# lesliegaga/GPT-SoVITS

Hardware: AMD Instinct MI355X
Metric: synthesised audio sec/sec (1/RTF), v2 pipeline (higher is better)
Workload: dtype f16

## Files before the change

gpt-sovits_amd/csrc/attn.hip:

```cpp
#include <stdlib.h>

#include "common.h"

#define GSV_PIN() do { asm volatile("" ::: "memory"); __builtin_amdgcn_sched_barrier(0); } while (0)

namespace gsv {

__device__ __forceinline__ f4 mma16(h8 a, h8 b, f4 c) { return __builtin_amdgcn_mfma_f32_16x16x32_f16(a, b, c, 0, 0, 0); }

__global__ __launch_bounds__(256) void vt_kernel(const _Float16* __restrict__ v, int ld, int T, int ldv, _Float16* __restrict__ vt,
                                                 int heads, _Float16* __restrict__ q, int ldq, _Float16* __restrict__ k, int ldk,
                                                 const float* __restrict__ rope_cs, int rope_half, int planes, long long xz,
                                                 long long vtz) {
  const int row = blockIdx.z / planes, plane = blockIdx.z - row * planes;
  v += row * xz; q += row * xz; k += row * xz; vt += row * vtz;
  if (plane == heads) {
    const int n = T * rope_half * 2;
    const int stride = gridDim.x * gridDim.y * 256;
    for (int i = (blockIdx.y * gridDim.x + blockIdx.x) * 256 + threadIdx.x; i < n; i += stride) {
      const int which = i / (T * rope_half);
      const int rr = i - which * T * rope_half;
      const int t = rr / rope_half, p = rr - t * rope_half;
      _Float16* x = (which ? k + (long long)t * ldk : q + (long long)t * ldq) + 2 * p;
      const float c = rope_cs[((long long)t * rope_half + p) * 2], sn = rope_cs[((long long)t * rope_half + p) * 2 + 1];
// ... 315 lines not shown
      den += e * Ls[w * BQ + qq];
      acc += *(const f4*)&Os[((size_t)w * BQ + qq) * LDO + d4] * e;
    }
#pragma unroll
    for (int rr = 0; rr < NB; ++rr) {
      const float pw = __expf(Sb[qq * NB + rr] - mt);
      const f4 rv = *(const f4*)(rel_v + rr * D + d4);
      acc += rv * pw;
    }
    const float inv = 1.f / den;
    *(h4*)(out + (long long)(q0 + qq) * ldo + head * D + d4) =
        (h4){(_Float16)(acc[0] * inv), (_Float16)(acc[1] * inv), (_Float16)(acc[2] * inv), (_Float16)(acc[3] * inv)};
  }
}

int launch_flash_rel96_f16(const void* q, int ldq, const void* k, int ldk, const void* v, int ldvv, void* vt_buf, int T, int heads,
                           float scale, const float* rel_k, const float* rel_v, void* out, int ldo, hipStream_t s, const int* kr) {
  GSV_REQUIRE(T >= 1 && heads >= 1 && rel_k && rel_v, "flash_rel96: bad argument");
  GSV_REQUIRE(ldq % 8 == 0 && ldk % 8 == 0 && ldo % 4 == 0 && ((uintptr_t)q % 16) == 0 && ((uintptr_t)k % 16) == 0 && ((uintptr_t)out % 8) == 0 &&
              ((uintptr_t)rel_v % 16) == 0, "flash_rel96: operands must be 16-byte aligned with leading dims multiple of 8");
  const int ldv = (T + 31) / 32 * 32;
  hipLaunchKernelGGL(vt96_kernel, dim3(ldv / 32, 3, heads), dim3(256), 0, s, (const _Float16*)v, ldvv, T, ldv, (_Float16*)vt_buf);
  constexpr int QT = 2;
  const size_t lds = ((size_t)4 * 16 * QT * 100 + 8 * 16 * QT + 2 * 16 * QT * 9) * 4;
  static bool attr = false;
  if (!attr) {
    GSV_HIP(hipFuncSetAttribute((const void*)flash_rel96_f16_kernel<QT>, hipFuncAttributeMaxDynamicSharedMemorySize, (int)lds));
    attr = true;
  }
  hipLaunchKernelGGL(flash_rel96_f16_kernel<QT>, dim3(cdiv(T, 16 * QT), heads), dim3(256), lds, s, (const _Float16*)q, ldq,
                     (const _Float16*)k, ldk, (const _Float16*)vt_buf, ldv, T, scale, rel_k, rel_v, (_Float16*)out, ldo, kr);
  GSV_HIP(hipGetLastError());
  return GSV_OK;
}

// ... 27 lines not shown
```

gpt-sovits_amd/csrc/engine.h:

```cpp
#pragma once
#include <math.h>
#include <map>
#include <string>
#include <vector>

#include "common.h"

struct Conv {
  void* w = nullptr;
  float* b = nullptr;
  int cin = 0, cout = 0, taps = 1;
  int ups_u = 0, ups_pad = 0, ups_cout = 0;
};

struct AttnLayerW { Conv qkv, o; float *rel_k = nullptr, *rel_v = nullptr; float *g1 = nullptr, *b1 = nullptr, *g2 = nullptr, *b2 = nullptr; Conv f1, f2; };
struct WNW { std::vector<Conv> in, res; std::vector<float*> in_bias_eff; Conv cond; };
struct FlowW { Conv pre, post; WNW wn; };

struct VocAct { float *alpha = nullptr, *beta = nullptr; };
struct GenW {
  int uic = 0, n_ups = 0, n_resblocks = 0;
  int up_rates[8], up_kernels[8], rb_kernels[4], rb_dilations[4][3];
  std::vector<Conv> ups, rb1, rb2;
  std::vector<VocAct> acts;
  int snake_logscale = 0;
  float *up12 = nullptr, *dn12 = nullptr;
};

struct Buf { void* p = nullptr; size_t cap = 0; };

struct gsv_vits {
  gsv_vits_config cfg;
// ... 91 lines not shown
```

gpt-sovits_amd/csrc/ops.hip:

```cpp
#include "common.h"

namespace gsv {

static thread_local char g_err[1024] = "";
void set_error(const char* fmt, ...) {
  va_list ap;
  va_start(ap, fmt);
  vsnprintf(g_err, sizeof(g_err), fmt, ap);
  va_end(ap);
}
const char* get_error() { return g_err; }

static thread_local unsigned long long g_conv_route = 0;
static thread_local unsigned long long g_pair_route = 0;
void set_conv_route(unsigned long long code) {
  g_conv_route = code;
  if ((code & 255) == ROUTE_CONV_PAIR) g_pair_route = code;
}

template <typename T> __global__ void convert_kernel(const float* __restrict__ s, T* __restrict__ d, long long n) {
  long long i = (long long)blockIdx.x * blockDim.x + threadIdx.x;
  long long stride = (long long)gridDim.x * blockDim.x;
  for (; i < n; i += stride) d[i] = (T)s[i];
}
// ... 219 lines not shown
                     float eps, int dtype, gsv_stream_t stream) {
  return gsv::launch_layernorm(dtype, x, 0, res, 0, gamma, beta, y, 0, rows, C, eps, (hipStream_t)stream);
}

int gsv_op_flash_attn64(const void* qkv, int T, int heads, float scale, void* vt_scratch, void* out, gsv_stream_t stream) {
  const int inner = heads * 64;
  return gsv::launch_flash_attn64_f16(qkv, 3 * inner, (const _Float16*)qkv + inner, 3 * inner, (const _Float16*)qkv + 2 * inner, 3 * inner,
                                      vt_scratch, T, heads, scale, out, inner, (hipStream_t)stream);
}

int gsv_op_flash_rel96(const void* qkv, int T, int heads, float scale, const float* rel_k, const float* rel_v, void* vt_scratch,
                       void* out, gsv_stream_t stream) {
  const int H = heads * 96;
  return gsv::launch_flash_rel96_f16(qkv, 3 * H, (const _Float16*)qkv + H, 3 * H, (const _Float16*)qkv + 2 * H, 3 * H, vt_scratch, T, heads,
                                     scale, rel_k, rel_v, out, H, (hipStream_t)stream);
}

int gsv_op_conv1d(const gsv_conv_desc* d, int dtype, gsv_stream_t stream) {
  gsv::ConvArgs a;
  a.x = d->x; a.w = d->w; a.bias = d->bias; a.y = d->y; a.res = d->res; a.gate = d->gate;
  a.T_in = d->T_in; a.T_out = d->T_out; a.Cin = d->Cin; a.Cout = d->Cout; a.taps = d->taps;
  a.stride = d->stride; a.dil = d->dil; a.pad = d->pad;
  a.ldx = d->Cin; a.ldw = d->taps * d->Cin;
  a.pre_act = d->pre_act; a.pre_slope = d->pre_slope; a.post_act = d->post_act; a.scale = d->scale;
  a.accumulate = d->accumulate; a.out_f32 = d->out_f32;
  a.res_f32 = d->res_dtype == 0 ? d->out_f32 : d->res_dtype == 1;
  a.y_col0 = d->y_col0; a.w_nt = d->w_nt; a.z_res = d->z_res;
  if (d->ups_u > 0) {
    a.ups_u = d->ups_u; a.ups_pad = d->ups_pad; a.ups_cout = d->Cout / d->ups_u;
    a.ldy = a.ups_cout; a.ldr = a.ups_cout;
// ... 88 lines not shown
```

gpt-sovits_amd/csrc/vits.hip:

```cpp
#include "engine.h"

namespace gsv {

template <typename T>
__global__ void gather_rows_kernel(const int* __restrict__ idx, const float* __restrict__ table, int C, int rep, int n,
                                   T* __restrict__ out) {
  const int row = blockIdx.x;
  if (row >= n * rep) return;
  const float* src = table + (long long)idx[row / rep] * C;
  T* dst = out + (long long)row * C;
  for (int c = threadIdx.x; c < C; c += blockDim.x) dst[c] = (T)src[c];
}

template <typename T>
__global__ void gather_seg_kernel(const int* __restrict__ ids, const int* __restrict__ src, const float* __restrict__ table, int C,
                                  int rows, T* __restrict__ out) {
  const int row = blockIdx.x;
  if (row >= rows) return;
  const int i = src[row];
  T* dst = out + (long long)row * C;
  if (i < 0) { for (int c = threadIdx.x; c < C; c += blockDim.x) dst[c] = (T)0.f; return; }
  const float* sp = table + (long long)ids[i] * C;
  for (int c = threadIdx.x; c < C; c += blockDim.x) dst[c] = (T)sp[c];
}
// ... 170 lines not shown
__global__ void gate_kernel(const T* __restrict__ a, long long n, int H, T* __restrict__ out) {
  long long i = (long long)blockIdx.x * blockDim.x + threadIdx.x;
  if (i >= n) return;
  long long t = i / H; int c = (int)(i - t * H);
  float x = to_f(a[t * 2 * H + c]), y = to_f(a[t * 2 * H + H + c]);
  out[i] = (T)(tanhf(x) * (1.f / (1.f + expf(-y))));
}

template <typename T>
__global__ void glu_res_kernel(const T* __restrict__ y, long long n, int H, T* __restrict__ x) {
  long long i = (long long)blockIdx.x * blockDim.x + threadIdx.x;
  if (i >= n) return;
  long long t = i / H; int c = (int)(i - t * H);
  float a = to_f(y[t * 2 * H + c]), b = to_f(y[t * 2 * H + H + c]);
  x[i] = (T)(to_f(x[i]) + a * (1.f / (1.f + expf(-b))));
}

template <typename T>
__global__ void flip_channels_kernel(const T* __restrict__ src, long long n, int C, T* __restrict__ dst) {
  long long i = (long long)blockIdx.x * blockDim.x + threadIdx.x;
  if (i >= n) return;
  long long t = i / C; int c = (int)(i - t * C);
  dst[i] = src[t * C + (C - 1 - c)];
}

__device__ __forceinline__ unsigned long long mix64(unsigned long long x) {
  x += 0x9E3779B97F4A7C15ull;
  x = (x ^ (x >> 30)) * 0xBF58476D1CE4E5B9ull;
  x = (x ^ (x >> 27)) * 0x94D049BB133111EBull;
  return x ^ (x >> 31);
}

template <typename T>
__global__ void zp_kernel(const float* __restrict__ stats, int F, int C, const float* __restrict__ noise, float scale,
                          unsigned long long seed, T* __restrict__ z, const int* __restrict__ seg, const int* __restrict__ start,
                          const int* __restrict__ noff, const unsigned long long* __restrict__ seeds, int Fn) {
  long long i = (long long)blockIdx.x * blockDim.x + threadIdx.x;
  if (i >= (long long)F * C) return;
// ... 646 lines not shown
  {
    std::vector<float> e;
    if (!fetch(h, "quantizer.vq.layers.0._codebook.embed", (size_t)c.n_bins * SSL, c.n_bins, e)) return GSV_ERR_ARG;
    GSV_RC(up_f32(h, e.data(), e.size(), &h->codebook));
    GSV_RC(up_t(h, e, &h->codebook_t));
    std::vector<float> ee(c.n_bins);
    for (int j = 0; j < c.n_bins; ++j) {
      float s = 0.f;
      for (int k = 0; k < SSL; ++k) s += e[(size_t)j * SSL + k] * e[(size_t)j * SSL + k];
      ee[j] = s;
    }
    GSV_RC(up_f32(h, ee.data(), ee.size(), &h->code_ee));
    GSV_RC(make_conv(h, "ssl_proj", SSL, SSL, 2, true, &h->top_ssl_proj));
  }
  if (c.flavor == 0) {
    for (int fi = 0; fi < 4; ++fi) {
      FlowW& f = h->flows[fi];
      const std::string p = "flow.flows." + std::to_string(2 * fi);
      GSV_RC(make_conv(h, p + ".pre", H, IC / 2, 1, true, &f.pre));
      GSV_RC(make_conv(h, p + ".post", IC / 2, H, 1, true, &f.post));
      GSV_RC(make_wn(h, p + ".enc", 4, H, GIN, &f.wn));
    }
    const int UIC = c.upsample_initial_channel;
    GSV_RC(make_conv(h, "dec.conv_pre", UIC, IC, 7, true, &h->conv_pre));
    GSV_RC(make_conv(h, "dec.cond", UIC, GIN, 1, true, &h->cond));
    GSV_RC(dalloc(h, (void**)&h->conv_pre_bias_eff, (size_t)UIC * 4));
    gen_shape(c, &h->gen);
    GSV_RC(load_generator(h, "dec.", false, &h->gen));
    GSV_RC(make_conv(h, "dec.conv_post", 1, UIC >> c.n_ups, 7, false, &h->conv_post));
  } else {
    const int W = 512, NL = 8;
    GSV_REQUIRE(IC == H, "vits: v3/v4 need inter_channels == hidden_channels (bridge = Conv1d(inter, 512) on the hidden sequence)");
    GSV_RC(make_conv(h, "bridge.0", W, IC, 1, true, &h->bridge));
    GSV_RC(make_conv(h, "wns1.pre", W, W, 1, true, &h->w1_pre));
    GSV_RC(make_conv(h, "wns1.proj", W, W, 1, true, &h->w1_proj));
// ... 65 lines not shown
}

template <typename T>
static int decode_wav(gsv_vits* h, hipStream_t s, const int32_t* codes, int Tc, const int32_t* phones, int L, double speed,
                      const float* noise, float noise_scale, uint64_t seed, float* wav, const SegRun* sr) {
  const auto& c = h->cfg;
  void* y = nullptr;
  int F = 0;
  GSV_RC(run_enc_p<T>(h, s, codes, Tc, phones, L, speed, &y, &F, sr));
  const size_t es = sizeof(T);
  const int H = c.hidden_channels, IC = c.inter_channels;
  const int* seg_f = sr ? sr->seg_p : nullptr;
  float* stats;
  GSV_RC(need(h, "stats", (size_t)F * 2 * IC * 4, (void**)&stats));
  { ConvOpt of; of.out_f32 = 1; GSV_RC(conv(h, s, h->proj, y, H, F, stats, F, of)); }
  void *z, *zf, *hb, *xin, *acts, *wout;
  GSV_RC(need(h, "z", (size_t)F * IC * es, &z));
  GSV_RC(need(h, "zf", (size_t)F * IC * es, &zf));
  GSV_RC(need(h, "wn_h", (size_t)F * H * es, &hb));
  GSV_RC(need(h, "wn_xin", (size_t)F * 2 * H * es, &xin));
  GSV_RC(need(h, "wn_acts", (size_t)F * H * es, &acts));
  GSV_RC(need(h, "wn_out", (size_t)F * H * es, &wout));
  GSV_LAUNCH(zp_kernel<T>, dim3(nblk((long long)F * IC)), dim3(256), 0, s, stats, F, IC, noise, noise_scale, (unsigned long long)seed, (T*)z,
             seg_f, sr ? sr->start : nullptr, sr ? sr->noff : nullptr, sr ? sr->seeds : nullptr, sr ? sr->post->Fn : 0);
  const int half = IC / 2;
  for (int fi = 3; fi >= 0; --fi) {
    FlowW& f = h->flows[fi];
    GSV_LAUNCH(flip_channels_kernel<T>, dim3(nblk((long long)F * IC)), dim3(256), 0, s, (const T*)z, (long long)F * IC, IC, (T*)zf);
    std::swap(z, zf);
    ConvOpt om; om.row_seg = seg_f;
    GSV_RC(conv(h, s, f.pre, z, IC, F, hb, F, om));
    GSV_RC(run_wn<T>(h, s, f.wn, F, hb, xin, acts, wout, sr, h->voice_off_in + (size_t)fi * 4 * 2 * H, F));
    ConvOpt op; op.scale = -1.f; op.accumulate = 1; op.ldy = IC; op.y_col0 = half; op.row_seg = seg_f;
    GSV_RC(conv(h, s, f.post, wout, H, F, z, F, op));
  }
  h->lastF = F;
  {
    void* zkeep;
    GSV_RC(need(h, "z_keep", (size_t)F * IC * es, &zkeep));
    GSV_HIP(hipMemcpyAsync(zkeep, z, (size_t)F * IC * es, hipMemcpyDeviceToDevice, s));
  }
  GSV_HIP(hipEventRecord(h->ev[1], s));
  void* gb[5];
  GSV_RC(gen_buffers(h, h->gen, "g", F, gb));
  void* cur = gb[3];
  GSV_RC(conv_voice(h, s, h->conv_pre, z, F, cur, ConvOpt(), h->conv_pre_bias_eff, sr, h->voice_off_pre, seg_f));
  int Tn = F;
  GSV_RC(run_generator_stages(h, s, h->gen, gb, &cur, &Tn, seg_f ? sr->seg_up.data() : nullptr));
  float* wout_p = wav;
  if (seg_f) GSV_RC(need(h, "wav_pad", (size_t)Tn * 4, (void**)&wout_p));
  { ConvOpt op; op.pre_act = ACT_LRELU; op.pre_slope = 0.01f; op.post_act = ACT_TANH; op.out_f32 = 1;
    GSV_RC(conv(h, s, h->conv_post, cur, h->conv_post.cin, Tn, wout_p, Tn, op)); }
  if (seg_f) {
    const int up = Tn / F;
    GSV_RC(launch_compact_wav(s, wout_p, seg_f, up, (long long)sr->post->G * up, (long long)Tn, wav));
  }
// ... 75 lines not shown
  GSV_REQUIRE(h && h->finalized, "vits_decode: handle not finalized");
  GSV_REQUIRE(h->has_ref, "vits_decode: call gsv_vits_set_refer first");
  GSV_REQUIRE(codes && phones && wav && Tc >= 1 && L >= 1, "vits_decode: empty input (T=%d, L=%d)", Tc, L);
  hipStream_t s = (hipStream_t)stream;
  GSV_REQUIRE(speed > 0.0, "vits_decode: speed must be positive");
  GSV_REQUIRE(h->cfg.flavor == 0, "vits_decode: this handle is a v3/v4 model (use gsv_vits_decode_encp + gsv_cfm_inference + a vocoder)");
  GSV_HIP(hipEventRecord(h->ev[0], s));
  return GSV_WITH_T(h, decode_wav<T>(h, s, codes, Tc, phones, L, speed, noise, noise_scale, seed, wav, nullptr));
}

int gsv_vits_segment_gap(const gsv_vits_config* cfg) {
  if (!cfg || cfg->n_ups < 1 || cfg->n_ups > 8 || cfg->n_resblocks < 1 || cfg->n_resblocks > 4) return -1;
  return seg_gap(*cfg);
}

int gsv_vits_segment_map(const gsv_vits_config* cfg, int n, const int* code_lens, const int* phone_lens, int level, int32_t* seg,
                         int64_t cap, int64_t* rows) {
  return gsv_vits_segment_map_speed(cfg, n, code_lens, phone_lens, nullptr, level, seg, cap, rows);
}

int gsv_vits_segment_map_speed(const gsv_vits_config* cfg, int n, const int* code_lens, const int* phone_lens, const double* speeds,
                               int level, int32_t* seg, int64_t cap, int64_t* rows) {
  GSV_REQUIRE(cfg && rows && cfg->n_ups >= 1 && cfg->n_ups <= 8, "vits_segment_map: bad argument");
  GSV_REQUIRE(level >= -1 && level <= cfg->n_ups, "vits_segment_map: level %d outside [-1, %d]", level, cfg->n_ups);
  SegLayout lay;
  GSV_RC(seg_layout(*cfg, n, code_lens, phone_lens, speeds, &lay));
  long long up = 1;
  for (int i = 0; i < level; ++i) up *= cfg->up_rates[i];
  const long long nr = level < 0 ? lay.L : (long long)lay.F * up;
  *rows = nr;
// ... 169 lines not shown
  }
  GSV_REQUIRE(F > 0, "vits_debug_tensor: no decode yet");
  if (n == "gen_last_in") {
    const long long ne = (long long)h->dbg_last_T * h->dbg_last_C;
    GSV_REQUIRE(h->dbg_last_in && cap >= ne, "vits_debug_tensor: buffer too small");
    *numel = ne;
    return GSV_WITH_T(h, debug_cl_to_cf<T>(s, h->dbg_last_in, h->dbg_last_T, h->dbg_last_C, out));
  }
  GSV_REQUIRE(cap >= (int64_t)F * IC, "vits_debug_tensor: buffer too small");
  *numel = (int64_t)F * IC;
  if (n == "m_p" || n == "logs_p") {
    const float* st = (const float*)h->bufs["stats"].p;
    GSV_LAUNCH(cl_to_cf_kernel<float>, dim3(nblk((long long)F * IC)), dim3(256), 0, s, st, F, 2 * IC, n == "m_p" ? 0 : IC, IC, out);
    return GSV_OK;
  }
  if (n == "z") return GSV_WITH_T(h, debug_cl_to_cf<T>(s, h->bufs["z_keep"].p, F, IC, out));
  set_error("vits_debug_tensor: unknown tensor '%s' (ge, m_p, logs_p, z, gen_last_in)", name);
  return GSV_ERR_ARG;
}

}
```

gpt-sovits_amd/gsv/_lib.py:

```python
from __future__ import annotations

import ctypes as C
import os

HERE = os.path.dirname(os.path.abspath(__file__))
LIB_PATH = os.path.join(HERE, "libgsv_hip.so")

GSV_F32, GSV_F16 = 0, 1


class T2SConfig(C.Structure):
    _fields_ = [(n, C.c_int) for n in ("n_layer", "dim", "n_head", "ffn_dim", "vocab", "phoneme_vocab", "bert_dim")]


class SamplingParams(C.Structure):
    _fields_ = [("top_k", C.c_int), ("top_p", C.c_float), ("temperature", C.c_float),
                ("repetition_penalty", C.c_float), ("early_stop_num", C.c_int), ("eos_mask_steps", C.c_int),
                ("max_steps", C.c_int), ("seed", C.c_uint64)]


class RowSampling(C.Structure):
    _fields_ = [("top_k", C.c_int), ("top_p", C.c_float), ("temperature", C.c_float), ("repetition_penalty", C.c_float)]


# ... 74 lines not shown
    "gsv_vits_debug_tensor": (C.c_int, [C.c_void_p, C.c_char_p, C.c_void_p, C.c_int64, C.POINTER(C.c_int64),
                                        C.c_void_p]),
    "gsv_vits_last_timing": (C.c_int, [C.c_void_p, C.POINTER(C.c_float), C.POINTER(C.c_float)]),
    "gsv_vits_store_voice": (C.c_int, [C.c_void_p, C.c_int]),
    "gsv_vits_decode_segments": (C.c_int, [C.c_void_p, C.c_int, C.c_void_p, C.POINTER(C.c_int), C.c_void_p, C.POINTER(C.c_int),
                                           C.POINTER(C.c_int), C.POINTER(C.c_uint64), C.c_void_p, C.c_float, C.c_void_p,
                                           C.c_void_p]),
    "gsv_vits_decode_segments_speed": (C.c_int, [C.c_void_p, C.c_int, C.c_void_p, C.POINTER(C.c_int), C.c_void_p, C.POINTER(C.c_int),
                                                 C.POINTER(C.c_int), C.POINTER(C.c_uint64), C.POINTER(C.c_double), C.c_void_p,
                                                 C.c_float, C.c_void_p, C.c_void_p]),
    "gsv_vits_segment_gap": (C.c_int, [C.POINTER(VitsConfig)]),
    "gsv_vits_segment_map": (C.c_int, [C.POINTER(VitsConfig), C.c_int, C.POINTER(C.c_int), C.POINTER(C.c_int), C.c_int,
                                       C.POINTER(C.c_int32), C.c_int64, C.POINTER(C.c_int64)]),
    "gsv_vits_segment_map_speed": (C.c_int, [C.POINTER(VitsConfig), C.c_int, C.POINTER(C.c_int), C.POINTER(C.c_int),
                                             C.POINTER(C.c_double), C.c_int, C.POINTER(C.c_int32), C.c_int64, C.POINTER(C.c_int64)]),
    "gsv_vocoder_create": (C.c_int, [C.POINTER(VocoderConfig), C.c_int, C.POINTER(C.c_void_p)]),
    "gsv_vocoder_destroy": (None, [C.c_void_p]),
    "gsv_vocoder_load_tensor": (C.c_int, [C.c_void_p, C.c_char_p, C.c_void_p, C.c_int64]),
    "gsv_vocoder_finalize": (C.c_int, [C.c_void_p]),
    "gsv_vocoder_forward": (C.c_int, [C.c_void_p, C.c_void_p, C.c_int, C.c_void_p, C.c_void_p]),
    "gsv_vocoder_forward_segments": (C.c_int, [C.c_void_p, C.c_void_p, C.c_int, C.POINTER(C.c_int), C.c_void_p, C.c_void_p]),
    "gsv_vocoder_segment_gap": (C.c_int, [C.POINTER(VocoderConfig)]),
    "gsv_vocoder_segment_map": (C.c_int, [C.POINTER(VocoderConfig), C.c_int, C.POINTER(C.c_int), C.c_int, C.POINTER(C.c_int32),
                                          C.c_int64]),
    "gsv_cfm_create": (C.c_int, [C.POINTER(DitConfig), C.c_int, C.POINTER(C.c_void_p)]),
    "gsv_cfm_destroy": (None, [C.c_void_p]),
    "gsv_cfm_load_tensor": (C.c_int, [C.c_void_p, C.c_char_p, C.c_void_p, C.c_int64]),
    "gsv_cfm_finalize": (C.c_int, [C.c_void_p]),
    "gsv_cfm_inference": (C.c_int, [C.c_void_p, C.c_void_p, C.c_void_p, C.c_int, C.c_int, C.c_int, C.c_int, C.c_void_p,
                                    C.c_float, C.c_uint64, C.c_void_p, C.c_void_p]),
# ... 14 lines not shown
    "gsv_postprocess": (C.c_int, [C.POINTER(C.c_void_p), C.POINTER(C.c_int), C.c_int, C.c_int, C.c_int, C.c_void_p, C.c_void_p]),
    "gsv_postprocess_f32": (C.c_int, [C.POINTER(C.c_void_p), C.POINTER(C.c_int), C.c_int, C.c_int, C.c_int, C.c_void_p,
                                      C.c_void_p]),
    "gsv_bwe_create": (C.c_int, [C.POINTER(BweConfig), C.c_int, C.POINTER(C.c_void_p)]),
    "gsv_bwe_destroy": (None, [C.c_void_p]),
    "gsv_bwe_load_tensor": (C.c_int, [C.c_void_p, C.c_char_p, C.c_void_p, C.c_int64]),
    "gsv_bwe_finalize": (C.c_int, [C.c_void_p]),
    "gsv_bwe_out_len": (C.c_int, [C.c_void_p, C.c_int, C.c_int]),
    "gsv_bwe_forward": (C.c_int, [C.c_void_p, C.c_void_p, C.c_int, C.c_int, C.c_int, C.c_void_p, C.c_void_p]),
    "gsv_bwe_debug_tensor": (C.c_int, [C.c_void_p, C.c_char_p, C.c_void_p, C.c_int64, C.POINTER(C.c_int64), C.c_void_p]),
    "gsv_aa_act_forward": (C.c_int, [C.c_void_p, C.c_void_p, C.c_void_p, C.c_void_p, C.c_void_p, C.c_void_p,
                                     C.c_int, C.c_int, C.c_int, C.c_int, C.c_void_p]),
    "gsv_op_flash_attn64": (C.c_int, [C.c_void_p, C.c_int, C.c_int, C.c_float, C.c_void_p, C.c_void_p, C.c_void_p]),
    "gsv_op_flash_rel96": (C.c_int, [C.c_void_p, C.c_int, C.c_int, C.c_float, C.c_void_p, C.c_void_p, C.c_void_p, C.c_void_p,
                                     C.c_void_p]),
    "gsv_op_conv1d": (C.c_int, [C.POINTER(ConvDesc), C.c_int, C.c_void_p]),
    "gsv_debug_last_conv_route": (C.c_uint64, [C.c_int]),
    "gsv_debug_last_pair_route": (C.c_uint64, [C.c_int]),
    "gsv_op_frame": (C.c_int, [C.c_void_p, C.c_int, C.c_int, C.c_int, C.c_int, C.c_int, C.c_int, C.c_void_p, C.c_int, C.c_void_p]),
    "gsv_op_magnitude": (C.c_int, [C.c_void_p, C.c_int, C.c_int, C.c_float, C.c_int, C.c_void_p, C.c_void_p]),
    "gsv_op_conv_pair": (C.c_int, [C.c_void_p, C.c_void_p, C.c_void_p, C.c_void_p, C.c_void_p, C.c_void_p, C.c_int, C.c_int, C.c_int,
                                  C.c_int, C.c_float, C.c_int, C.c_void_p]),
    "gsv_op_conv_pair_seg": (C.c_int, [C.c_void_p, C.c_void_p, C.c_void_p, C.c_void_p, C.c_void_p, C.c_void_p, C.c_int, C.c_int, C.c_int,
                                      C.c_int, C.c_float, C.c_int, C.c_void_p, C.c_void_p]),
    "gsv_op_aa_act_cl": (C.c_int, [C.c_void_p, C.c_void_p, C.c_int, C.c_int, C.c_void_p, C.c_void_p, C.c_int, C.c_void_p, C.c_void_p,
                                  C.c_void_p, C.c_int, C.c_int, C.c_void_p]),
    "gsv_op_aff_mix": (C.c_int, [C.c_void_p, C.c_void_p, C.c_void_p, C.c_longlong, C.c_void_p, C.c_void_p]),
    "gsv_op_time_mean": (C.c_int, [C.c_void_p, C.c_int, C.c_int, C.c_void_p, C.c_void_p]),
    "gsv_op_channel_norm": (C.c_int, [C.c_void_p, C.c_int, C.c_int, C.c_void_p, C.c_void_p, C.c_float, C.c_int, C.c_void_p,
                                      C.c_void_p, C.c_int, C.c_void_p]),
# ... 62 lines not shown
```

include/gsv.h:

```cpp
#ifndef GSV_H_
#define GSV_H_

#include <stdint.h>

#ifdef __cplusplus
extern "C" {
#endif

#define GSV_OK 0
#define GSV_ERR_ARG (-1)
#define GSV_ERR_HIP (-2)
#define GSV_ERR_STATE (-3)

#define GSV_F32 0
#define GSV_F16 1

typedef void* gsv_stream_t;

int gsv_init(int device);
const char* gsv_last_error(void);
int gsv_abi_version(void);

typedef struct gsv_t2s gsv_t2s_t;

// ... 85 lines not shown
int gsv_vits_set_refer_sv(gsv_vits_t* h, const float* const* specs, const int* frames, int bins, const float* const* sv_embs,
                          int n_refs, gsv_stream_t stream);
#define GSV_VITS_MAX_VOICES 128
int gsv_vits_store_voice(gsv_vits_t* h, int slot);
int gsv_vits_decode_segments(gsv_vits_t* h, int n, const int32_t* codes, const int* code_lens, const int32_t* phones,
                             const int* phone_lens, const int* voice_slots, const uint64_t* seeds, const float* noise,
                             float noise_scale, float* wav, gsv_stream_t stream);
int gsv_vits_decode_segments_speed(gsv_vits_t* h, int n, const int32_t* codes, const int* code_lens, const int32_t* phones,
                                   const int* phone_lens, const int* voice_slots, const uint64_t* seeds, const double* speeds,
                                   const float* noise, float noise_scale, float* wav, gsv_stream_t stream);
int gsv_vits_segment_gap(const gsv_vits_config* cfg);
int gsv_vits_segment_map(const gsv_vits_config* cfg, int n, const int* code_lens, const int* phone_lens, int level, int32_t* seg,
                         int64_t cap, int64_t* rows);
int gsv_vits_segment_map_speed(const gsv_vits_config* cfg, int n, const int* code_lens, const int* phone_lens, const double* speeds,
                               int level, int32_t* seg, int64_t cap, int64_t* rows);
int gsv_vits_last_timing(gsv_vits_t* h, float* total_ms, float* generator_ms);

typedef struct gsv_vocoder gsv_vocoder_t;

typedef struct {
  int kind;
  int in_channels;
  int upsample_initial_channel;
  int n_ups;
  int up_rates[8];
  int up_kernels[8];
  int n_resblocks;
  int rb_kernels[4];
  int rb_dilations[4][3];
  int bias_at_final;
// ... 70 lines not shown
  int T_in, T_out, Cin, Cout, taps, stride, dil, pad;
  int pre_act; float pre_slope; int post_act; float scale; int accumulate; int out_f32;
  int ups_u, ups_pad;
  int Z; long long xz, wz, yz; int ldx, ldw, ldy;
  const float* gate;
  int bz;
  long long rz; int ldr;
  int res_dtype;
  int y_col0;
  int w_nt;
  int z_res;
} gsv_conv_desc;
int gsv_op_flash_attn64(const void* qkv, int T, int heads, float scale, void* vt_scratch, void* out, gsv_stream_t stream);
int gsv_op_flash_rel96(const void* qkv, int T, int heads, float scale, const float* rel_k, const float* rel_v, void* vt_scratch,
                       void* out, gsv_stream_t stream);
int gsv_op_decode_attn(const void* q, const void* kc, const void* vc, const int32_t* kv_len, const int32_t* active, int B, int H,
                       int smax, int dtype, void* out, gsv_stream_t stream);
int gsv_op_conv1d(const gsv_conv_desc* d, int dtype, gsv_stream_t stream);
uint64_t gsv_debug_last_conv_route(int reset);
uint64_t gsv_debug_last_pair_route(int reset);
int gsv_op_layernorm(const void* x, const void* res, const float* gamma, const float* beta, void* y, int rows,
                     int C, float eps, int dtype, gsv_stream_t stream);
int gsv_op_lora_delta(const void* x, void* y, int Tn, int DB, int K, int N, int n_proj, const int* slots, int n_slots,
                      const void* const* blocks, const int* rp, const float* gate, int dtype, gsv_stream_t stream);
int gsv_op_frame(const float* x, int n, int frame_len, int hop, int pad, int ld, int T_out, void* out, int dtype, gsv_stream_t stream);
int gsv_op_magnitude(const float* re_im, int T, int bins, float eps, int frame_ld, float* spec, gsv_stream_t stream);
int gsv_op_conv_pair(const void* x, const void* w1, const float* b1, const void* w2, const float* b2, void* y, int T, int C, int taps,
                     int dil, float scale, int accumulate, gsv_stream_t stream);
int gsv_op_conv_pair_seg(const void* x, const void* w1, const float* b1, const void* w2, const float* b2, void* y, int T, int C, int taps,
                         int dil, float scale, int accumulate, const int32_t* row_seg, gsv_stream_t stream);
// ... 19 lines not shown
```

Measured before the change: 2835.

## Add tiled rel96 flash kernel, drop flow channel flips, remove z copy

Result: no change. 2862 (median of 2 runs) (+0.9%).

```diff
diff --git a/gpt-sovits_amd/csrc/attn.hip b/gpt-sovits_amd/csrc/attn.hip
--- a/gpt-sovits_amd/csrc/attn.hip
+++ b/gpt-sovits_amd/csrc/attn.hip
@@ -353,11 +353,269 @@
   }
 }
 
+namespace rel96 {
+constexpr int D = 96, KS = 3, ND = 6, W = 4, NB = 9, LDO = 100;
+constexpr int QT = 2, QG = 2, KSPL = 4;
+constexpr int BQ = 16 * QT * QG;
+constexpr int KB = 32 * KSPL;
+constexpr int NT = 64 * QG * KSPL;
+constexpr int LDK = D + 8, LDV = KB + 8;
+constexpr int STAGE = KB * LDK + D * LDV;
+constexpr int KLOADS = KB * (D / 8) / NT;
+constexpr int VTHREADS = (KB / 4) * (D / 8);
+constexpr size_t LDS_BYTES = (size_t)2 * STAGE * 2 + ((size_t)2 * KSPL * BQ + 2 * BQ * NB) * 4;
+static_assert(KB * (D / 8) % NT == 0 && VTHREADS % 64 == 0 && VTHREADS <= NT, "rel96: staging does not divide");
+static_assert((size_t)KSPL * BQ * LDO * 4 <= (size_t)2 * STAGE * 2, "rel96: the combine buffer must fit in the stage buffers");
+}
+
+__device__ __forceinline__ float qmax4(float x) {
+  const unsigned u = __float_as_uint(x);
+  const auto a = __builtin_amdgcn_permlane16_swap(u, u, false, false);
+  const unsigned w = __float_as_uint(fmaxf(__uint_as_float(a[0]), __uint_as_float(a[1])));
+  const auto b = __builtin_amdgcn_permlane32_swap(w, w, false, false);
+  return fmaxf(__uint_as_float(b[0]), __uint_as_float(b[1]));
+}
+
+template <bool SEG>
+__global__ __launch_bounds__(rel96::NT) void flash_rel96_tiled_f16_kernel(const _Float16* __restrict__ q, int ldq,
+                                                                          const _Float16* __restrict__ k, int ldk,
+                                                                          const _Float16* __restrict__ v, int ldv, int T, float scale,
+                                                                          const float* __restrict__ rel_k, const float* __restrict__ rel_v,
+                                                                          _Float16* __restrict__ out, int ldo, const int* __restrict__ kr) {
+  using namespace rel96;
+  extern __shared__ float smem[];
+  _Float16* stage = (_Float16*)smem;
+  float* Os = smem;
+  float* Ms = smem + STAGE;
+  float* Ls = Ms + KSPL * BQ;
+  float* Bias = Ls + KSPL * BQ;
+  float* Sb = Bias + BQ * NB;
+  const int vid = xcd_virtual_id(blockIdx.y * gridDim.x + blockIdx.x, gridDim.x * gridDim.y);
+  const int head = vid / gridDim.x, q0 = (vid % gridDim.x) * BQ;
+  const int tid = threadIdx.x, lane = tid & 63, wave = tid >> 6;
+  const int qg = wave / KSPL, ksp = wave % KSPL;
+  const int r = lane & 15, g = lane >> 4;
+  const int lq0 = 32 * qg;
+  const float sc2 = scale * 1.44269504088896341f;
+  h8 qf[QT][KS];
+#pragma unroll
+  for (int t = 0; t < QT; ++t) {
+    const _Float16* qp = q + (long long)min(q0 + lq0 + 16 * t + r, T - 1) * ldq + head * D + g * 8;
+#pragma unroll
+    for (int ks = 0; ks < KS; ++ks) qf[t][ks] = *(const h8*)(qp + 32 * ks);
+  }
+  for (int i = tid; i < BQ * NB; i += NT) Sb[i] = -INFINITY;
+#pragma unroll
+  for (int t = 0; t < QT; ++t) {
+    if (t != ksp) continue;
+#pragma unroll
+    for (int rr = 0; rr < NB; ++rr) {
+      float sdot = 0.f;
+#pragma unroll
+      for (int ks = 0; ks < KS; ++ks)
+#pragma unroll
+        for (int e = 0; e < 8; ++e) sdot += (float)qf[t][ks][e] * rel_k[rr * D + ks * 32 + g * 8 + e];
+      sdot += __shfl_xor(sdot, 16, 64);
+      sdot += __shfl_xor(sdot, 32, 64);
+      if (g == 0) Bias[(lq0 + 16 * t + r) * NB + rr] = sdot * sc2;
+    }
+  }
+#pragma unroll
+  for (int t = 0; t < QT; ++t)
+#pragma unroll
+    for (int ks = 0; ks < KS; ++ks)
+#pragma unroll
+      for (int e = 0; e < 8; ++e) qf[t][ks][e] = (_Float16)((float)qf[t][ks][e] * sc2);
+  int klo[QT], khi[QT];
+#pragma unroll
+  for (int t = 0; t < QT; ++t) {
+    const int qi = min(q0 + lq0 + 16 * t + r, T - 1);
+    klo[t] = SEG ? kr[2 * qi] : 0;
+    khi[t] = SEG ? kr[2 * qi + 1] : T;
+  }
+  const int glo = SEG ? max(kr[2 * q0], 0) : 0, ghi = SEG ? min(kr[2 * min(q0 + BQ - 1, T - 1) + 1], T) : T;
+  const int wlo = SEG ? max(kr[2 * min(q0 + lq0, T - 1)], 0) : 0, whi = SEG ? min(kr[2 * min(q0 + lq0 + 31, T - 1) + 1], T) : T;
+  const int s0 = glo / KB, ns = (ghi + KB - 1) / KB;
+  f4 o[QT][ND];
+  float m[QT], l[QT];
+#pragma unroll
+  for (int t = 0; t < QT; ++t) {
+    m[t] = -INFINITY; l[t] = 0.f;
+#pragma unroll
+    for (int d = 0; d < ND; ++d) o[t][d] = (f4){0.f, 0.f, 0.f, 0.f};
+  }
+  struct KVR { h8 k[KLOADS], v[4]; };
+  const _Float16* kg = k + head * D;
+  const _Float16* vg = v + head * D;
+  const int vkq = tid & (KB / 4 - 1), vc = tid / (KB / 4);
+  auto gload = [&](KVR& f, int st) {
+    const int key0 = st * KB;
+#pragma unroll
+    for (int i = 0; i < KLOADS; ++i) {
+      const int idx = tid + NT * i, key = idx / (D / 8), c = idx - key * (D / 8);
+      f.k[i] = *(const h8*)(kg + (long long)min(key0 + key, T - 1) * ldk + 8 * c);
+    }
+    if (tid < VTHREADS) {
+#pragma unroll
+      for (int i = 0; i < 4; ++i) {
+        const int j = key0 + 4 * vkq + i;
+        f.v[i] = *(const h8*)(vg + (long long)min(j, T - 1) * ldv + 8 * vc);
+      }
+    }
+  };
+  auto lstore = [&](const KVR& f, _Float16* buf) {
+#pragma unroll
+    for (int i = 0; i < KLOADS; ++i) {
+      const int idx = tid + NT * i, key = idx / (D / 8), c = idx - key * (D / 8);
+      const int j = key & 31;
+      const int row = (key & ~31) + ((j >> 2) & 1) * 16 + 4 * (j >> 3) + (j & 3);
+      *(h8*)(buf + row * LDK + 8 * c) = f.k[i];
+    }
+    if (tid < VTHREADS) {
+      _Float16* vt = buf + KB * LDK + (8 * vc) * LDV + 4 * vkq;
+#pragma unroll
+      for (int e = 0; e < 8; ++e) *(h4*)(vt + e * LDV) = (h4){f.v[0][e], f.v[1][e], f.v[2][e], f.v[3][e]};
+    }
+  };
+  auto process = [&](const _Float16* buf, int key0, bool mask) {
+    const _Float16* kp = buf + (32 * ksp + r) * LDK + 8 * g;
+    const _Float16* vp = buf + KB * LDK + r * LDV + 32 * ksp + 8 * g;
+    h8 ka[KS], kb[KS], vf[ND];
+#pragma unroll
+    for (int ks = 0; ks < KS; ++ks) { ka[ks] = *(const h8*)(kp + 32 * ks); kb[ks] = *(const h8*)(kp + 16 * LDK + 32 * ks); }
+#pragma unroll
+    for (int d = 0; d < ND; ++d) vf[d] = *(const h8*)(vp + 16 * d * LDV);
+#pragma unroll
+    for (int t = 0; t < QT; ++t) {
+      f4 sa = (f4){0.f, 0.f, 0.f, 0.f}, sb = sa;
+#pragma unroll
+      for (int ks = 0; ks < KS; ++ks) { sa = mma16(ka[ks], qf[t][ks], sa); sb = mma16(kb[ks], qf[t][ks], sb); }
+      float p[8];
+#pragma unroll
+      for (int i = 0; i < 4; ++i) { p[i] = sa[i]; p[4 + i] = sb[i]; }
+      if (SEG || mask) {
+#pragma unroll
+        for (int i = 0; i < 8; ++i) {
+          const int j = key0 + 8 * g + i;
+          p[i] = (j >= klo[t] && j < khi[t]) ? p[i] : -INFINITY;
+        }
+      }
+      const int qt0 = q0 + lq0 + 16 * t;
+      if (key0 + 31 >= qt0 - W && key0 <= qt0 + 15 + W) {
+        const int qi = qt0 + r;
+#pragma unroll
+        for (int i = 0; i < 8; ++i) {
+          const int j = key0 + 8 * g + i;
+          const int rp = j - qi + W;
+          if (rp >= 0 && rp < NB && qi < T && j >= klo[t] && j < khi[t]) {
+            p[i] += Bias[(lq0 + 16 * t + r) * NB + rp];
+            Sb[(lq0 + 16 * t + r) * NB + rp] = p[i];
+          }
+        }
+      }
+      float mx = -INFINITY;
+#pragma unroll
+      for (int i = 0; i < 8; ++i) mx = fmaxf(mx, p[i]);
+      mx = qmax4(mx);
+      if (__any(mx > m[t])) {
+        const float mnew = fmaxf(m[t], mx);
+        const float alpha = __builtin_amdgcn_exp2f(m[t] - mnew);
+        l[t] *= (m[t] == mnew) ? 1.f : alpha;
+#pragma unroll
+        for (int d = 0; d < ND; ++d) o[t][d] *= (m[t] == mnew) ? 1.f : alpha;
+        m[t] = mnew;
+      }
+      const float msafe = m[t] == -INFINITY ? 0.f : m[t];
+#pragma unroll
+      for (int i = 0; i < 8; ++i) p[i] = __builtin_amdgcn_exp2f(p[i] - msafe);
+      const h8 pf = (h8){(_Float16)p[0], (_Float16)p[1], (_Float16)p[2], (_Float16)p[3], (_Float16)p[4], (_Float16)p[5], (_Float16)p[6], (_Float16)p[7]};
+#pragma unroll
+      for (int d = 0; d < ND; ++d) o[t][d] = mma16(vf[d], pf, o[t][d]);
+      l[t] += ((p[0] + p[1]) + (p[2] + p[3])) + ((p[4] + p[5]) + (p[6] + p[7]));
+    }
+  };
+  KVR fA, fB;
+  gload(fA, s0);
+  lstore(fA, stage);
+  if (s0 + 1 < ns) gload(fA, s0 + 1);
+  __syncthreads();
+  auto run_stage = [&](int st, const KVR& mine, KVR& other) {
+    _Float16* cur = stage + ((st - s0) & 1) * STAGE;
+    _Float16* nxt = stage + ((st - s0 + 1) & 1) * STAGE;
+    if (st + 2 < ns) gload(other, st + 2);
+    GSV_PIN();
+    const int key0 = st * KB + 32 * ksp;
+    if (key0 + 32 > wlo && key0 < whi) process(cur, key0, st == ns - 1);
+    GSV_PIN();
+    if (st + 1 < ns) lstore(mine, nxt);
+    __syncthreads();
+  };
+  for (int st = s0; st < ns; st += 2) {
+    run_stage(st, fA, fB);
+    if (st + 1 < ns) run_stage(st + 1, fB, fA);
+  }
+#pragma unroll
+  for (int t = 0; t < QT; ++t) {
+#pragma unroll
+    for (int d = 0; d < ND; ++d) *(f4*)&Os[((size_t)ksp * BQ + lq0 + 16 * t + r) * LDO + d * 16 + 4 * g] = o[t][d];
+    float lt = l[t];
+    lt += __shfl_xor(lt, 16, 64);
+    lt += __shfl_xor(lt, 32, 64);
+    if (g == 0) { Ms[ksp * BQ + lq0 + 16 * t + r] = m[t]; Ls[ksp * BQ + lq0 + 16 * t + r] = lt; }
+  }
+  __syncthreads();
+  for (int it = tid; it < BQ * (D / 4); it += NT) {
+    const int qq = it / (D / 4), d4 = (it % (D / 4)) * 4;
+    if (q0 + qq >= T) continue;
+    const float mt = fmaxf(fmaxf(Ms[qq], Ms[BQ + qq]), fmaxf(Ms[2 * BQ + qq], Ms[3 * BQ + qq]));
+    float den = 0.f;
+    f4 acc = (f4){0.f, 0.f, 0.f, 0.f};
+#pragma unroll
+    for (int w = 0; w < KSPL; ++w) {
+      const float e = __builtin_amdgcn_exp2f(Ms[w * BQ + qq] - mt);
+      den += e * Ls[w * BQ + qq];
+      acc += *(const f4*)&Os[((size_t)w * BQ + qq) * LDO + d4] * e;
+    }
+#pragma unroll
+    for (int rr = 0; rr < NB; ++rr) {
+      const float pw = __builtin_amdgcn_exp2f(Sb[qq * NB + rr] - mt);
+      const f4 rv = *(const f4*)(rel_v + rr * D + d4);
+      acc += rv * pw;
+    }
+    const float inv = 1.f / den;
+    *(h4*)(out + (long long)(q0 + qq) * ldo + head * D + d4) =
+        (h4){(_Float16)(acc[0] * inv), (_Float16)(acc[1] * inv), (_Float16)(acc[2] * inv), (_Float16)(acc[3] * inv)};
+  }
+}
+
+template <bool SEG>
+static int launch_flash_rel96_tiled(const void* q, int ldq, const void* k, int ldk, const void* v, int ldvv, int T, int heads, float scale,
+                                    const float* rel_k, const float* rel_v, void* out, int ldo, hipStream_t s, const int* kr) {
+  static bool attr = false;
+  if (!attr) {
+    GSV_HIP(hipFuncSetAttribute((const void*)flash_rel96_tiled_f16_kernel<SEG>, hipFuncAttributeMaxDynamicSharedMemorySize,
+                                (int)rel96::LDS_BYTES));
+    attr = true;
+  }
+  hipLaunchKernelGGL(flash_rel96_tiled_f16_kernel<SEG>, dim3(cdiv(T, rel96::BQ), heads), dim3(rel96::NT), rel96::LDS_BYTES, s,
+                     (const _Float16*)q, ldq, (const _Float16*)k, ldk, (const _Float16*)v, ldvv, T, scale, rel_k, rel_v, (_Float16*)out, ldo, kr);
+  GSV_HIP(hipGetLastError());
+  return GSV_OK;
+}
+
 int launch_flash_rel96_f16(const void* q, int ldq, const void* k, int ldk, const void* v, int ldvv, void* vt_buf, int T, int heads,
                            float scale, const float* rel_k, const float* rel_v, void* out, int ldo, hipStream_t s, const int* kr) {
   GSV_REQUIRE(T >= 1 && heads >= 1 && rel_k && rel_v, "flash_rel96: bad argument");
   GSV_REQUIRE(ldq % 8 == 0 && ldk % 8 == 0 && ldo % 4 == 0 && ((uintptr_t)q % 16) == 0 && ((uintptr_t)k % 16) == 0 && ((uintptr_t)out % 8) == 0 &&
               ((uintptr_t)rel_v % 16) == 0, "flash_rel96: operands must be 16-byte aligned with leading dims multiple of 8");
+  static const bool v1 = getenv("GSV_FLASH_REL96_V1") && atoi(getenv("GSV_FLASH_REL96_V1")) != 0;
+  if (!v1) {
+    GSV_REQUIRE(ldvv % 8 == 0 && ((uintptr_t)v % 16) == 0, "flash_rel96: v must be 16-byte aligned with a leading dim multiple of 8");
+    GSV_REQUIRE(heads <= 65535, "flash_rel96: %d heads exceed the grid", heads);
+    if (kr) return launch_flash_rel96_tiled<true>(q, ldq, k, ldk, v, ldvv, T, heads, scale, rel_k, rel_v, out, ldo, s, kr);
+    return launch_flash_rel96_tiled<false>(q, ldq, k, ldk, v, ldvv, T, heads, scale, rel_k, rel_v, out, ldo, s, kr);
+  }
+  GSV_REQUIRE(vt_buf, "flash_rel96: the first-generation kernel needs its V^T scratch");
   const int ldv = (T + 31) / 32 * 32;
   hipLaunchKernelGGL(vt96_kernel, dim3(ldv / 32, 3, heads), dim3(256), 0, s, (const _Float16*)v, ldvv, T, ldv, (_Float16*)vt_buf);
   constexpr int QT = 2;
diff --git a/gpt-sovits_amd/csrc/engine.h b/gpt-sovits_amd/csrc/engine.h
--- a/gpt-sovits_amd/csrc/engine.h
+++ b/gpt-sovits_amd/csrc/engine.h
@@ -15,7 +15,7 @@
 
 struct AttnLayerW { Conv qkv, o; float *rel_k = nullptr, *rel_v = nullptr; float *g1 = nullptr, *b1 = nullptr, *g2 = nullptr, *b2 = nullptr; Conv f1, f2; };
 struct WNW { std::vector<Conv> in, res; std::vector<float*> in_bias_eff; Conv cond; };
-struct FlowW { Conv pre, post; WNW wn; };
+struct FlowW { Conv pre, post, pre_r, post_r; WNW wn; };
 
 struct VocAct { float *alpha = nullptr, *beta = nullptr; };
 struct GenW {
diff --git a/gpt-sovits_amd/csrc/ops.hip b/gpt-sovits_amd/csrc/ops.hip
--- a/gpt-sovits_amd/csrc/ops.hip
+++ b/gpt-sovits_amd/csrc/ops.hip
@@ -257,6 +257,13 @@
   const int H = heads * 96;
   return gsv::launch_flash_rel96_f16(qkv, 3 * H, (const _Float16*)qkv + H, 3 * H, (const _Float16*)qkv + 2 * H, 3 * H, vt_scratch, T, heads,
                                      scale, rel_k, rel_v, out, H, (hipStream_t)stream);
+}
+
+int gsv_op_flash_rel96_seg(const void* qkv, int T, int heads, float scale, const float* rel_k, const float* rel_v, void* vt_scratch,
+                           void* out, const int32_t* kr, gsv_stream_t stream) {
+  const int H = heads * 96;
+  return gsv::launch_flash_rel96_f16(qkv, 3 * H, (const _Float16*)qkv + H, 3 * H, (const _Float16*)qkv + 2 * H, 3 * H, vt_scratch, T, heads,
+                                     scale, rel_k, rel_v, out, H, (hipStream_t)stream, kr);
 }
 
 int gsv_op_conv1d(const gsv_conv_desc* d, int dtype, gsv_stream_t stream) {
diff --git a/gpt-sovits_amd/csrc/vits.hip b/gpt-sovits_amd/csrc/vits.hip
--- a/gpt-sovits_amd/csrc/vits.hip
+++ b/gpt-sovits_amd/csrc/vits.hip
@@ -208,14 +208,6 @@
   long long t = i / H; int c = (int)(i - t * H);
   float a = to_f(y[t * 2 * H + c]), b = to_f(y[t * 2 * H + H + c]);
   x[i] = (T)(to_f(x[i]) + a * (1.f / (1.f + expf(-b))));
-}
-
-template <typename T>
-__global__ void flip_channels_kernel(const T* __restrict__ src, long long n, int C, T* __restrict__ dst) {
-  long long i = (long long)blockIdx.x * blockDim.x + threadIdx.x;
-  if (i >= n) return;
-  long long t = i / C; int c = (int)(i - t * C);
-  dst[i] = src[t * C + (C - 1 - c)];
 }
 
 __device__ __forceinline__ unsigned long long mix64(unsigned long long x) {
@@ -892,11 +884,25 @@
     GSV_RC(make_conv(h, "ssl_proj", SSL, SSL, 2, true, &h->top_ssl_proj));
   }
   if (c.flavor == 0) {
+    GSV_REQUIRE((IC / 2 * esz(h)) % 16 == 0, "vits: inter_channels / 2 must keep the upper half of z 16-byte aligned");
     for (int fi = 0; fi < 4; ++fi) {
       FlowW& f = h->flows[fi];
       const std::string p = "flow.flows." + std::to_string(2 * fi);
       GSV_RC(make_conv(h, p + ".pre", H, IC / 2, 1, true, &f.pre));
       GSV_RC(make_conv(h, p + ".post", IC / 2, H, 1, true, &f.post));
+      if (fi & 1) {
+        const int half = IC / 2;
+        std::vector<float> pw, pb, qw, qb;
+        if (!fetch(h, p + ".pre.weight", (size_t)H * half, H, pw) || !fetch(h, p + ".pre.bias", H, H, pb) ||
+            !fetch(h, p + ".post.weight", (size_t)half * H, half, qw) || !fetch(h, p + ".post.bias", half, half, qb))
+          return GSV_ERR_ARG;
+        std::vector<float> pwr(pw.size()), qwr(qw.size()), qbr(qb.size());
+        GSV_RC(gsv_vits_flow_reversed_operands(H, half, pw.data(), qw.data(), qb.data(), pwr.data(), qwr.data(), qbr.data()));
+        h->staged[p + ".pre_r.weight"] = pwr; h->staged[p + ".pre_r.bias"] = pb;
+        h->staged[p + ".post_r.weight"] = qwr; h->staged[p + ".post_r.bias"] = qbr;
+        GSV_RC(make_conv(h, p + ".pre_r", H, half, 1, true, &f.pre_r));
+        GSV_RC(make_conv(h, p + ".post_r", half, H, 1, true, &f.post_r));
+      }
       GSV_RC(make_wn(h, p + ".enc", 4, H, GIN, &f.wn));
     }
     const int UIC = c.upsample_initial_channel;
@@ -992,9 +998,8 @@
   float* stats;
   GSV_RC(need(h, "stats", (size_t)F * 2 * IC * 4, (void**)&stats));
   { ConvOpt of; of.out_f32 = 1; GSV_RC(conv(h, s, h->proj, y, H, F, stats, F, of)); }
-  void *z, *zf, *hb, *xin, *acts, *wout;
+  void *z, *hb, *xin, *acts, *wout;
   GSV_RC(need(h, "z", (size_t)F * IC * es, &z));
-  GSV_RC(need(h, "zf", (size_t)F * IC * es, &zf));
   GSV_RC(need(h, "wn_h", (size_t)F * H * es, &hb));
   GSV_RC(need(h, "wn_xin", (size_t)F * 2 * H * es, &xin));
   GSV_RC(need(h, "wn_acts", (size_t)F * H * es, &acts));
@@ -1002,22 +1007,19 @@
   GSV_LAUNCH(zp_kernel<T>, dim3(nblk((long long)F * IC)), dim3(256), 0, s, stats, F, IC, noise, noise_scale, (unsigned long long)seed, (T*)z,
              seg_f, sr ? sr->start : nullptr, sr ? sr->noff : nullptr, sr ? sr->seeds : nullptr, sr ? sr->post->Fn : 0);
   const int half = IC / 2;
+  bool rev = false;
   for (int fi = 3; fi >= 0; --fi) {
     FlowW& f = h->flows[fi];
-    GSV_LAUNCH(flip_channels_kernel<T>, dim3(nblk((long long)F * IC)), dim3(256), 0, s, (const T*)z, (long long)F * IC, IC, (T*)zf);
-    std::swap(z, zf);
+    rev = !rev;
+    GSV_REQUIRE(!rev || (f.pre_r.w && f.post_r.w), "vits: flow %d has no reversed operands", fi);
     ConvOpt om; om.row_seg = seg_f;
-    GSV_RC(conv(h, s, f.pre, z, IC, F, hb, F, om));
+    GSV_RC(conv(h, s, rev ? f.pre_r : f.pre, (const T*)z + (rev ? half : 0), IC, F, hb, F, om));
     GSV_RC(run_wn<T>(h, s, f.wn, F, hb, xin, acts, wout, sr, h->voice_off_in + (size_t)fi * 4 * 2 * H, F));
-    ConvOpt op; op.scale = -1.f; op.accumulate = 1; op.ldy = IC; op.y_col0 = half; op.row_seg = seg_f;
-    GSV_RC(conv(h, s, f.post, wout, H, F, z, F, op));
-  }
+    ConvOpt op; op.scale = -1.f; op.accumulate = 1; op.ldy = IC; op.y_col0 = rev ? 0 : half; op.row_seg = seg_f;
+    GSV_RC(conv(h, s, rev ? f.post_r : f.post, wout, H, F, z, F, op));
+  }
+  GSV_REQUIRE(!rev, "vits: the flow must leave z in its logical channel order");
   h->lastF = F;
-  {
-    void* zkeep;
-    GSV_RC(need(h, "z_keep", (size_t)F * IC * es, &zkeep));
-    GSV_HIP(hipMemcpyAsync(zkeep, z, (size_t)F * IC * es, hipMemcpyDeviceToDevice, s));
-  }
   GSV_HIP(hipEventRecord(h->ev[1], s));
   void* gb[5];
   GSV_RC(gen_buffers(h, h->gen, "g", F, gb));
@@ -1123,6 +1125,19 @@
   return seg_gap(*cfg);
 }
 
+int gsv_vits_flow_reversed_operands(int hidden, int half, const float* pre_w, const float* post_w, const float* post_b, float* pre_w_rev,
+                                    float* post_w_rev, float* post_b_rev) {
+  GSV_REQUIRE(hidden >= 1 && half >= 1 && pre_w && post_w && post_b && pre_w_rev && post_w_rev && post_b_rev,
+              "vits_flow_reversed_operands: bad argument");
+  for (int o = 0; o < hidden; ++o)
+    for (int j = 0; j < half; ++j) pre_w_rev[(size_t)o * half + j] = pre_w[(size_t)o * half + (half - 1 - j)];
+  for (int j = 0; j < half; ++j) {
+    for (int i = 0; i < hidden; ++i) post_w_rev[(size_t)j * hidden + i] = post_w[(size_t)(half - 1 - j) * hidden + i];
+    post_b_rev[j] = post_b[half - 1 - j];
+  }
+  return GSV_OK;
+}
+
 int gsv_vits_segment_map(const gsv_vits_config* cfg, int n, const int* code_lens, const int* phone_lens, int level, int32_t* seg,
                          int64_t cap, int64_t* rows) {
   return gsv_vits_segment_map_speed(cfg, n, code_lens, phone_lens, nullptr, level, seg, cap, rows);
@@ -1322,7 +1337,7 @@
     GSV_LAUNCH(cl_to_cf_kernel<float>, dim3(nblk((long long)F * IC)), dim3(256), 0, s, st, F, 2 * IC, n == "m_p" ? 0 : IC, IC, out);
     return GSV_OK;
   }
-  if (n == "z") return GSV_WITH_T(h, debug_cl_to_cf<T>(s, h->bufs["z_keep"].p, F, IC, out));
+  if (n == "z") return GSV_WITH_T(h, debug_cl_to_cf<T>(s, h->bufs["z"].p, F, IC, out));
   set_error("vits_debug_tensor: unknown tensor '%s' (ge, m_p, logs_p, z, gen_last_in)", name);
   return GSV_ERR_ARG;
 }
diff --git a/gpt-sovits_amd/gsv/_lib.py b/gpt-sovits_amd/gsv/_lib.py
--- a/gpt-sovits_amd/gsv/_lib.py
+++ b/gpt-sovits_amd/gsv/_lib.py
@@ -112,6 +112,7 @@
                                        C.POINTER(C.c_int32), C.c_int64, C.POINTER(C.c_int64)]),
     "gsv_vits_segment_map_speed": (C.c_int, [C.POINTER(VitsConfig), C.c_int, C.POINTER(C.c_int), C.POINTER(C.c_int),
                                              C.POINTER(C.c_double), C.c_int, C.POINTER(C.c_int32), C.c_int64, C.POINTER(C.c_int64)]),
+    "gsv_vits_flow_reversed_operands": (C.c_int, [C.c_int, C.c_int] + [C.POINTER(C.c_float)] * 6),
     "gsv_vocoder_create": (C.c_int, [C.POINTER(VocoderConfig), C.c_int, C.POINTER(C.c_void_p)]),
     "gsv_vocoder_destroy": (None, [C.c_void_p]),
     "gsv_vocoder_load_tensor": (C.c_int, [C.c_void_p, C.c_char_p, C.c_void_p, C.c_int64]),
@@ -156,6 +157,8 @@
     "gsv_op_flash_attn64": (C.c_int, [C.c_void_p, C.c_int, C.c_int, C.c_float, C.c_void_p, C.c_void_p, C.c_void_p]),
     "gsv_op_flash_rel96": (C.c_int, [C.c_void_p, C.c_int, C.c_int, C.c_float, C.c_void_p, C.c_void_p, C.c_void_p, C.c_void_p,
                                      C.c_void_p]),
+    "gsv_op_flash_rel96_seg": (C.c_int, [C.c_void_p, C.c_int, C.c_int, C.c_float, C.c_void_p, C.c_void_p, C.c_void_p, C.c_void_p,
+                                         C.c_void_p, C.c_void_p]),
     "gsv_op_conv1d": (C.c_int, [C.POINTER(ConvDesc), C.c_int, C.c_void_p]),
     "gsv_debug_last_conv_route": (C.c_uint64, [C.c_int]),
     "gsv_debug_last_pair_route": (C.c_uint64, [C.c_int]),
diff --git a/include/gsv.h b/include/gsv.h
--- a/include/gsv.h
+++ b/include/gsv.h
@@ -123,6 +123,8 @@
                          int64_t cap, int64_t* rows);
 int gsv_vits_segment_map_speed(const gsv_vits_config* cfg, int n, const int* code_lens, const int* phone_lens, const double* speeds,
                                int level, int32_t* seg, int64_t cap, int64_t* rows);
+int gsv_vits_flow_reversed_operands(int hidden, int half, const float* pre_w, const float* post_w, const float* post_b, float* pre_w_rev,
+                                    float* post_w_rev, float* post_b_rev);
 int gsv_vits_last_timing(gsv_vits_t* h, float* total_ms, float* generator_ms);
 
 typedef struct gsv_vocoder gsv_vocoder_t;
@@ -223,6 +225,8 @@
 int gsv_op_flash_attn64(const void* qkv, int T, int heads, float scale, void* vt_scratch, void* out, gsv_stream_t stream);
 int gsv_op_flash_rel96(const void* qkv, int T, int heads, float scale, const float* rel_k, const float* rel_v, void* vt_scratch,
                        void* out, gsv_stream_t stream);
+int gsv_op_flash_rel96_seg(const void* qkv, int T, int heads, float scale, const float* rel_k, const float* rel_v, void* vt_scratch,
+                           void* out, const int32_t* kr, gsv_stream_t stream);
 int gsv_op_decode_attn(const void* q, const void* kc, const void* vc, const int32_t* kv_len, const int32_t* active, int B, int H,
                        int smax, int dtype, void* out, gsv_stream_t stream);
 int gsv_op_conv1d(const gsv_conv_desc* d, int dtype, gsv_stream_t stream);
```
